# NomaDamas/AutoRAG-Research

Measured on AMD Instinct MI355X. Metric: queries/sec, higher is better.
Workload: dtype f32

## Files before the change

autorag_research_amd/csrc/dev_common.h:

```cpp
#pragma once
#include <hip/hip_runtime.h>
#include <stdint.h>

namespace mi355 {

constexpr int kWave = 64;
constexpr int kQBlockMax = 1024;
constexpr int kKMax = 1024;
constexpr int kCandCap = 2048;
constexpr int kCandCapWide = 4096;
constexpr int kSortMax = 4096;
constexpr int kIrrCap = 1024;
constexpr uint64_t kKeyNaN = 0xFFFFFFFFFFFFFFFFull;
static_assert(kSortMax >= kKMax + kCandCap, "the general prune's sort must hold k kept entries and a full candidate list");

constexpr int kStOverflow = 1;
constexpr int kStIrregular = 2;

struct QueryState {
    float* qn;
    uint16_t* qhat;
    float* thr;
    int* cnt;
    int* best_n;
// ... 191 lines not shown
__device__ __forceinline__ void bitonic_asc_key_row(uint64_t* key, int32_t* row, int n) {
    for (int k = 2; k <= n; k <<= 1) {
        for (int j = k >> 1; j > 0; j >>= 1) {
            for (int i = threadIdx.x; i < n; i += blockDim.x) {
                const int p = i ^ j;
                if (p > i) {
                    const bool asc = ((i & k) == 0);
                    const uint64_t ka = key[i], kb = key[p];
                    const int32_t ra = row[i], rb = row[p];
                    const bool a_after_b = key_before(kb, rb, ka, ra);
                    if (asc ? a_after_b : key_before(ka, ra, kb, rb)) {
                        key[i] = kb;
                        key[p] = ka;
                        row[i] = rb;
                        row[p] = ra;
                    }
                }
            }
            __syncthreads();
        }
    }
}

constexpr int kStageCols = 64;
constexpr int kStageLd = 68;
constexpr int kStageFloats = kWave * kStageLd;

__device__ __forceinline__ void wave_sync() {
    __builtin_amdgcn_fence(__ATOMIC_RELEASE, "wavefront");
    __builtin_amdgcn_wave_barrier();
    __builtin_amdgcn_fence(__ATOMIC_ACQUIRE, "wavefront");
}

typedef float f32x4_native __attribute__((ext_vector_type(4)));
typedef const f32x4_native __attribute__((address_space(1)))* gmem_f4;
__device__ __forceinline__ float4 load_gmem_f4(const float* p) {
    const f32x4_native v = *(gmem_f4)p;
    return make_float4(v.x, v.y, v.z, v.w);
}

struct StagePiece {
    float4 v[16];
};
struct StageRows {
    const float* r[16];
};
__device__ __forceinline__ void stage_rows_init(StageRows& sr, const float* my_row, int lane) {
    const unsigned long long a = (unsigned long long)my_row;
    const unsigned plo = (unsigned)(a & 0xFFFFFFFFull), phi = (unsigned)(a >> 32);
    const int sub = lane >> 4;
#pragma unroll
    for (int g = 0; g < 16; ++g) {
        const unsigned lo = __shfl(plo, g * 4 + sub, kWave), hi = __shfl(phi, g * 4 + sub, kWave);
        sr.r[g] = (const float*)(((unsigned long long)hi << 32) | lo);
    }
}

__device__ __forceinline__ bool stage_rows_init_dense(StageRows& sr, const float* my_row, int lane) {
    const unsigned long long live = __builtin_amdgcn_ballot_w64(my_row != nullptr);
    if (live == 0) {
        stage_rows_init(sr, my_row, lane);
        return false;
    }
    const int src = __builtin_ctzll(live);
    unsigned long long a = (unsigned long long)my_row;
    unsigned plo = (unsigned)(a & 0xFFFFFFFFull), phi = (unsigned)(a >> 32);
    const unsigned flo = __shfl(plo, src, kWave), fhi = __shfl(phi, src, kWave);
    if (my_row == nullptr) {
        plo = flo;
        phi = fhi;
    }
    const int sub = lane >> 4;
#pragma unroll
    for (int g = 0; g < 16; ++g) {
        const unsigned lo = __shfl(plo, g * 4 + sub, kWave), hi = __shfl(phi, g * 4 + sub, kWave);
        sr.r[g] = (const float*)(((unsigned long long)hi << 32) | lo);
    }
    return true;
}
__device__ __forceinline__ void stage_issue_dense(StagePiece& p, const StageRows& sr, int k0, int lane) {
    const int c4 = (lane & 15) * 4;
#pragma unroll
    for (int g = 0; g < 16; ++g) p.v[g] = load_gmem_f4(sr.r[g] + k0 + c4);
}

__device__ __forceinline__ void stage_issue(StagePiece& p, const StageRows& sr, int k0, int d, int lane) {
    const int c4 = (lane & 15) * 4;
#pragma unroll
    for (int g = 0; g < 16; ++g)
        p.v[g] = (sr.r[g] != nullptr && k0 + c4 < d) ? load_gmem_f4(sr.r[g] + k0 + c4) : make_float4(0.f, 0.f, 0.f, 0.f);
}
__device__ __forceinline__ void stage_commit(float* tile, const StagePiece& p, int lane) {
    wave_sync();
    const int sub = lane >> 4, c4 = (lane & 15) * 4;
#pragma unroll
    for (int g = 0; g < 16; ++g) *(float4*)(tile + (g * 4 + sub) * kStageLd + c4) = p.v[g];
    wave_sync();
}

__device__ __forceinline__ void stage_rows(float* tile, const float* my_row, int k0, int d, int lane) {
    if ((d & 3) == 0) {
        StageRows sr;
        StagePiece p;
        stage_rows_init(sr, my_row, lane);
        stage_issue(p, sr, k0, d, lane);
        stage_commit(tile, p, lane);
        return;
    }
    wave_sync();
    const unsigned long long a = (unsigned long long)my_row;
    const unsigned plo = (unsigned)(a & 0xFFFFFFFFull), phi = (unsigned)(a >> 32);
#pragma unroll 8
    for (int s = 0; s < kWave; ++s) {
        const unsigned lo = __shfl(plo, s, kWave), hi = __shfl(phi, s, kWave);
        const float* r = (const float*)(((unsigned long long)hi << 32) | lo);
        const int k = k0 + lane;
        tile[s * kStageLd + lane] = (r != nullptr && k < d) ? r[k] : 0.0f;
    }
    wave_sync();
}

__device__ __forceinline__ float chain_piece(const float* tile, int lane, const float* qv, int kn, float acc) {
    const float* t = tile + lane * kStageLd;
    if (kn == kStageCols) {
        float4 tv[16], q4[16];
#pragma unroll
        for (int i = 0; i < 16; ++i) {
            tv[i] = *(const float4*)(t + 4 * i);
            q4[i] = *(const float4*)(qv + 4 * i);
        }
#pragma unroll
        for (int i = 0; i < 16; ++i) {
            acc = __builtin_fmaf(tv[i].x, q4[i].x, acc);
            acc = __builtin_fmaf(tv[i].y, q4[i].y, acc);
            acc = __builtin_fmaf(tv[i].z, q4[i].z, acc);
            acc = __builtin_fmaf(tv[i].w, q4[i].w, acc);
        }
        return acc;
    }
    int k = 0;
    for (; k + 4 <= kn; k += 4) {
        const float4 tv = *(const float4*)(t + k);
        const float4 q4 = *(const float4*)(qv + k);
        acc = __builtin_fmaf(tv.x, q4.x, acc);
        acc = __builtin_fmaf(tv.y, q4.y, acc);
        acc = __builtin_fmaf(tv.z, q4.z, acc);
        acc = __builtin_fmaf(tv.w, q4.w, acc);
    }
    for (; k < kn; ++k) acc = __builtin_fmaf(t[k], qv[k], acc);
    return acc;
}

#ifndef MI355_STAGE_DEPTH
#define MI355_STAGE_DEPTH 2
#endif
template <int DEPTH = MI355_STAGE_DEPTH>
__device__ __forceinline__ float staged_dot(float* tile, const float* my_row, const float* qv, int d, int lane) {
    static_assert(DEPTH == 2 || DEPTH == 3, "pieces in flight");
    float acc = 0.0f;
    if ((d & 3) == 0) {
        StageRows sr;
        StagePiece p0, p1, p2;
        const bool dense = stage_rows_init_dense(sr, my_row, lane);
        auto issue = [&](StagePiece& p, int k0) __attribute__((always_inline)) {
            if (dense && k0 + kStageCols <= d) stage_issue_dense(p, sr, k0, lane);
            else stage_issue(p, sr, k0, d, lane);
        };
        issue(p0, 0);
        if (kStageCols < d) issue(p1, kStageCols);
        if constexpr (DEPTH == 3) {
            if (2 * kStageCols < d) issue(p2, 2 * kStageCols);
        }
        for (int k0 = 0; k0 < d; k0 += DEPTH * kStageCols) {
            stage_commit(tile, p0, lane);
            if (k0 + DEPTH * kStageCols < d) issue(p0, k0 + DEPTH * kStageCols);
            acc = chain_piece(tile, lane, qv + k0, min(kStageCols, d - k0), acc);
            if (k0 + kStageCols < d) {
                stage_commit(tile, p1, lane);
                if (k0 + (DEPTH + 1) * kStageCols < d) issue(p1, k0 + (DEPTH + 1) * kStageCols);
                acc = chain_piece(tile, lane, qv + k0 + kStageCols, min(kStageCols, d - k0 - kStageCols), acc);
            }
            if constexpr (DEPTH == 3) {
                if (k0 + 2 * kStageCols < d) {
                    stage_commit(tile, p2, lane);
                    if (k0 + 5 * kStageCols < d) issue(p2, k0 + 5 * kStageCols);
                    acc = chain_piece(tile, lane, qv + k0 + 2 * kStageCols, min(kStageCols, d - k0 - 2 * kStageCols), acc);
                }
            }
        }
    } else {
        for (int k0 = 0; k0 < d; k0 += kStageCols) {
            stage_rows(tile, my_row, k0, d, lane);
            acc = chain_piece(tile, lane, qv + k0, min(kStageCols, d - k0), acc);
        }
    }
    return acc;
}

__device__ __forceinline__ float chain_piece16(const float* tile, int lane, const float* qv, int kn_words, float acc) {
    const float* t = tile + lane * kStageLd;
    for (int w = 0; w + 4 <= kn_words; w += 4) {
        const uint4 tv = *(const uint4*)(t + w);
        const float4 qa = *(const float4*)(qv + 2 * w), qb = *(const float4*)(qv + 2 * w + 4);
        acc = __builtin_fmaf(__uint_as_float(tv.x << 16), qa.x, acc);
        acc = __builtin_fmaf(__uint_as_float(tv.x & 0xFFFF0000u), qa.y, acc);
        acc = __builtin_fmaf(__uint_as_float(tv.y << 16), qa.z, acc);
        acc = __builtin_fmaf(__uint_as_float(tv.y & 0xFFFF0000u), qa.w, acc);
        acc = __builtin_fmaf(__uint_as_float(tv.z << 16), qb.x, acc);
        acc = __builtin_fmaf(__uint_as_float(tv.z & 0xFFFF0000u), qb.y, acc);
        acc = __builtin_fmaf(__uint_as_float(tv.w << 16), qb.z, acc);
        acc = __builtin_fmaf(__uint_as_float(tv.w & 0xFFFF0000u), qb.w, acc);
    }
    return acc;
}
__device__ __forceinline__ float staged_dot16(float* tile, const float* my_row_words, const float* qv, int words, int lane) {
    float acc = 0.0f;
    StageRows sr;
    StagePiece p0, p1;
    stage_rows_init(sr, my_row_words, lane);
    stage_issue(p0, sr, 0, words, lane);
    if (kStageCols < words) stage_issue(p1, sr, kStageCols, words, lane);
    for (int k0 = 0; k0 < words; k0 += 2 * kStageCols) {
        stage_commit(tile, p0, lane);
        if (k0 + 2 * kStageCols < words) stage_issue(p0, sr, k0 + 2 * kStageCols, words, lane);
        acc = chain_piece16(tile, lane, qv + 2 * k0, min(kStageCols, words - k0), acc);
        if (k0 + kStageCols < words) {
            stage_commit(tile, p1, lane);
            if (k0 + 3 * kStageCols < words) stage_issue(p1, sr, k0 + 3 * kStageCols, words, lane);
            acc = chain_piece16(tile, lane, qv + 2 * (k0 + kStageCols), min(kStageCols, words - k0 - kStageCols), acc);
        }
    }
    return acc;
}

}
```

autorag_research_amd/csrc/k_select.h:

```cpp
#pragma once
#include "dev_common.h"

namespace mi355 {

struct PruneArgs {
    const float* rows;
    const float* nrm2;
    const float* q;
    QueryState st;
    int32_t* cand_row;
    float* cand_val;
    const int* qlist;
    unsigned long long* stat;
    int cap, d, k, metric;
    int exact;
    const uint8_t* flag8;
    float cscale;
    const uint16_t* shadow16;
    int dpad;
    int round_a;
    int* skip_list;
    int skip_parity;
    int thr_only;
    int one_wave_only;
// ... 159 lines not shown
        a.stat[2 * q] += (unsigned long long)(n_new - a.st.carry[q]);
        a.st.carry[q] = 0;
    }

    int n_res;
    int n_base = n_best;
    bool kept_loaded = false;
    if constexpr (THREADS == kWave) {
        if (!a.exact) {
            float* tile = tiles;
            uint32_t key[kSelPerLane];
            unsigned in_a = 0;
            load_candidate_keys<kSelPerLane, kWave>(key, cval, crow, a.flag8, n_new, lane);
            for (int k = lane; k < a.d; k += kWave) qs[k] = a.q[(int64_t)q * a.d + k];
            if (a.shadow16 != nullptr)
                for (int k = lane; k < a.dpad; k += kWave) q16[k] = bf16_bits_to_f32(a.st.qhat[(int64_t)q * a.dpad + k]);
            const int n_cand = wave_count_ge(key, 1u, n_new);
            auto rescore_list = [&](int n, int dst) __attribute__((always_inline)) {
                for (int base = 0; base < n; base += kWave) {
                    const int e = base + lane;
                    const bool live = e < n;
                    const int32_t row = live ? crow[R[e]] : -1;
                    const float* rp = live ? a.rows + (int64_t)row * a.d : nullptr;
                    const float acc = staged_dot(tile, rp, qs, a.d, lane);
                    if (live) {
                        int32_t kept = row;
                        SK[dst + e] = exact_key_of(a.metric, acc, nq, a.nrm2[row], kept);
                        SR[dst + e] = kept;
                    }
                }
            };
            auto compact = [&](uint32_t x, int room, bool mark) -> int {
                int n = 0;
#pragma unroll
                for (int j = 0; j < kSelPerLane; ++j) {
                    if (j * kWave >= n_new) break;
                    const bool want = key[j] >= x && key[j] != 0 && !((in_a >> j) & 1u);
                    const unsigned long long bal = __builtin_amdgcn_ballot_w64(want);
                    const int pos = n + (int)__builtin_amdgcn_mbcnt_hi((unsigned)(bal >> 32),
                                                                       __builtin_amdgcn_mbcnt_lo((unsigned)bal, 0));
                    if (want && pos < room) {
                        R[pos] = j * kWave + lane;
                        if (mark) in_a |= 1u << j;
                    }
                    n += __builtin_popcountll(bal);
                }
                return min(n, room);
// ... 52 lines not shown
                        }
                    }
                    asm volatile("s_waitcnt vmcnt(0)" ::: "memory");
#pragma unroll
                    for (int j = 0; j < kSelPerLane; ++j) {
                        if (j * kWave >= nB) break;
                        const int i = j * kWave + lane;
                        if (i < nB) {
                            crow_w[i] = cr[j];
                            cval_w[i] = cv[j];
                        }
                    }
                    carried = nB;
                    nB = 0;
                }
                if (a.shadow16 != nullptr && cut16 != -__builtin_inff() && nB > 0) {
                    const int words = a.dpad / 2;
                    int nS = 0;
                    for (int base = 0; base < nB; base += kWave) {
                        const int e = base + lane;
                        const bool live = e < nB;
                        const int ci = live ? R[e] : 0;
                        const float* rp = live ? (const float*)(a.shadow16 + (int64_t)crow[ci] * a.dpad) : nullptr;
                        const float t16 = staged_dot16(tile, rp, q16, words, lane);
                        const bool keep = live && !(t16 < cut16);
                        const unsigned long long bal = __builtin_amdgcn_ballot_w64(keep);
                        const int pos = nS + (int)__builtin_amdgcn_mbcnt_hi((unsigned)(bal >> 32),
                                                                           __builtin_amdgcn_mbcnt_lo((unsigned)bal, 0));
                        wave_sync();
                        if (keep) R[pos] = ci;
                        nS += __builtin_popcountll(bal);
                    }
                    nB = nS;
                    wave_sync();
                }
                rescore_list(nB, n1);
            }
            if (lane == 0) a.stat[2 * q + 1] += (unsigned long long)(nA + nB);
            wave_sync();
            const int n_tot = n1 + nB;
            uint64_t* K2 = (uint64_t*)X;
            int32_t* R2 = (int32_t*)(X + (size_t)SORT * 8);
            int n_sel = n_tot;
            if (n_tot > a.k) {
                uint32_t sk[kSelPerLane];
#pragma unroll
                for (int j = 0; j < kSelPerLane; ++j) {
// ... 275 lines not shown
```

autorag_research_amd/csrc/mi355dr.hip:

```cpp
#include "index.h"
#include "k_prep.h"
#include "k_scan.h"
#include "k_scan_ids.h"
#include "subset_ids.h"
#include "screen_common.h"
#include "k_screen.h"
#include "k_screen256c.h"
#include "k_screen_rq.h"

#define MI355_RQ_FORMS(X) X(1) X(2) X(3) X(4) X(5) X(6)
inline bool screen_rq_has(int ksteps) { return ksteps >= 1 && ksteps <= 6; }
#include "k_screen_stream.h"
#include "k_select.h"
#include "k_prune_wide.h"
#include "k_update.h"
#include "k_compact.h"
#include "k_view.h"
#include "k_block.h"
#include "k_mmr.h"
#include "mmr_order.h"
#include "k_groups.h"
#include "k_range.h"
#include "k_rows.h"

// ... 195 lines not shown
}

inline bool i8_available(const mi355dr_index* idx) { return idx->irr8_n <= kIrrCap; }
Pass decide_pass(const mi355dr_index* idx, int k, int level, bool force_scan, const char* no_screen = nullptr) {
    Pass ps;
    ps.k = k;
    ps.level = level;
    const int path = force_scan ? (int)MI355DR_PATH_SCAN : idx->path;
    if (level > 0) ps.i8 = false;
    else if (idx->screen_dtype == MI355DR_SCREEN_I8) ps.i8 = true;
    else ps.i8 = idx->screen_dtype == MI355DR_SCREEN_AUTO && i8_available(idx) && k < idx->i8_demoted_k &&
                 growth_budget(idx, k, true) >= idx->i8_min_budget;
    const bool screen_possible = ps.i8 ? i8_available(idx) : idx->irr_n <= kIrrCap;
    ps.screening = idx->n > 0 && screen_possible && path != MI355DR_PATH_SCAN;
    ps.wide = ps.screening && wide_ok(idx, k);
    ps.cap = !idx->cap_set && ps.wide ? kCandCapWide : idx->cap;
    if (idx->screen_dtype == MI355DR_SCREEN_I8 && !i8_available(idx) && path != MI355DR_PATH_SCAN)
        ps.refused = "int8 screen unavailable: too many rows outside the residual limit";
    else if (path == MI355DR_PATH_SCREEN && !screen_possible && idx->n > 0) ps.refused = no_screen;
    return ps;
}
inline bool idle_i8(const mi355dr_index* idx) { return decide_pass(idx, idx->last_pass_k, 0, false).i8; }

int launch_prune(mi355dr_index* idx, hipStream_t s, const Pass& ps, int nblocks, const int* qlist, int exact,
                 bool thr_only = false, bool one_wave_only = false, bool defer_b = false) {
    PruneArgs pa{};
    pa.thr_only = thr_only ? 1 : 0;
    pa.one_wave_only = one_wave_only ? 1 : 0;
    pa.defer_b = defer_b && idx->defer_round_b ? 1 : 0;
    pa.rows = idx->rows;
    pa.nrm2 = idx->nrm2;
    pa.q = idx->qdev;
    pa.st = idx->st;
    pa.cand_row = idx->cand_row;
    pa.cand_val = idx->cand_val;
    pa.qlist = qlist;
    pa.stat = idx->stat_dev;
    pa.cap = ps.cap;
    pa.d = idx->dim;
    pa.k = ps.k;
    pa.metric = idx->metric;
    pa.exact = exact;
    pa.flag8 = (ps.i8 && (idx->irr8_n > 0 || idx->dead_n > 0)) ? idx->flag8 : nullptr;
    pa.cscale = idx->metric == MI355DR_METRIC_IP ? idx->cmax : 1.0f;
    pa.shadow16 = (ps.i8 && idx->metric == 0 && !exact && idx->prefilter16) ? idx->shadow : nullptr;
    pa.dpad = idx->dpad;
    pa.round_a = idx->round_a;
    if (!exact && ps.wide) {
        pa.shadow16 = nullptr;
        hipLaunchKernelGGL((k_prune_wide<2, 32>), dim3(nblocks), dim3(2 * kWave), prune_wide_lds_bytes(idx->dim, 2), s, pa);
        HIPCHECK(idx, hipGetLastError());
        return MI355DR_OK;
    }
    if (pa.cap > kCandCap) return fail(idx, MI355DR_E_INTERNAL, "general-form prune on a list stride above kCandCap");
    const bool list_mode = qlist == nullptr;
    pa.skip_list = list_mode ? idx->prune_skip : nullptr;
    pa.skip_parity = list_mode ? (idx->prune_parity ^= 1) : 0;
    hipLaunchKernelGGL((k_prune<kPruneSmallThreads, kPruneSmallSort>), dim3(nblocks), dim3(kPruneSmallThreads),
                       prune_lds_bytes(idx->dim, kPruneSmallThreads, kPruneSmallSort, pa.shadow16 ? idx->dpad : 0), s, pa);
    HIPCHECK(idx, hipGetLastError());
    if (one_wave_only) return MI355DR_OK;
    hipLaunchKernelGGL((k_prune<kPruneBigThreads, kPruneBigSort>), dim3(list_mode ? std::min(nblocks, 64) : nblocks),
                       dim3(kPruneBigThreads), prune_lds_bytes(idx->dim, kPruneBigThreads, kPruneBigSort, 0), s, pa);
    HIPCHECK(idx, hipGetLastError());
    return MI355DR_OK;
}

int launch_prep(mi355dr_index* idx, hipStream_t s, int B, int Bpad, int metric, bool i8, int cnt0 = 0) {
    hipLaunchKernelGGL(k_prep_queries, dim3(Bpad), dim3(64), (size_t)idx->dim * sizeof(float), s, idx->qdev, B, idx->dim,
                       idx->dpad, metric, idx->st, idx->dpad8, i8 ? 1 : 0, idx->bf16_ec, idx->status_or_dev,
                       idx->prune_skip, cnt0, idx->metric == MI355DR_METRIC_IP ? idx->cmax : 1.0f);
    idx->prune_parity = 0;
    HIPCHECK(idx, hipGetLastError());
    return MI355DR_OK;
}

inline int screen_tile(int B) { return B > kTileN ? kT2 : kTileM; }

constexpr int kRetryLevels = 2;

enum ScreenKernel { kKernTile = 0, kKernStream = 1, kKern256c = 2, kKernRq = 3 };
inline ScreenKernel screen_kernel_for(const mi355dr_index* idx, bool i8, int B, int64_t rows, bool emit_all) {
    const int tile = (emit_all || rows <= idx->small_chunk_rows) ? kTileM : screen_tile(B);
    const int row_bytes = i8 ? idx->dpad8 : idx->dpad * 2;
    const int ksteps = row_bytes / kRowB;
    if (tile == kT2) return i8 && idx->screen_rq && screen_rq_has(ksteps) ? kKernRq : kKern256c;
    if (!emit_all && idx->screen_stream && B <= 64 && ksteps >= 1 && (B <= 32 ? 32 : 64) * row_bytes <= kStreamQueryBytesMax)
        return kKernStream;
    return kKernTile;
}

int launch_screen(mi355dr_index* idx, hipStream_t s, bool i8, int B, int64_t r0, int64_t r_end, int cap, int emit_mode,
// ... 134 lines not shown
            const int64_t len = end - prev;
            if (len >= 2 * round_rows) end = std::min<int64_t>(n, prev + (len + round_rows / 2) / round_rows * round_rows);
        }
        if (end <= prev) continue;
        p.ends.push_back(end);
        prev = end;
        if (end >= n) break;
    }
    if (p.ends.empty() || p.ends.back() < n) p.ends.push_back(n);
    return p;
}

inline int starter_count(const PassPlan& p) { return (int)((p.sample + kSlabRows - 1) / kSlabRows); }

PassPlan make_plan(const mi355dr_index* idx, const Pass& ps, int B) {
    const double budget = growth_budget(idx, ps.k, ps.i8);
    double growth = std::max(0.25, std::min((double)idx->chunk_growth, budget));
    if (B <= 64 && ps.level == 0 && idx->chunk_growth_set == 0) growth = std::max(growth, std::min(8.0, budget * kSmallBlockBudget));
    if (ps.level == 1) growth = std::max(0.25, growth * 0.5);
    if (ps.level >= 2) growth = 0.25;
    return plan_pass(idx, ps, B, growth);
}

int run_screen(mi355dr_index* idx, hipStream_t s, const Pass& ps, int B, const PassPlan& plan) {
    int64_t kept_all_below = 0;
    const bool i8 = ps.i8;
    const int side_n = i8 ? idx->irr8_n : idx->irr_n;
    constexpr int kSideMerge = 32;
    bool side_done = false;
    const bool lean = plan.sample > 0 && idx->prune_companion == 0;
    auto timed = [&](bool big, int64_t rows, auto&& launch) -> int {
        EventPair ev{};
        if (idx->profile) {
            ev = take_events(idx);
            HIPCHECK(idx, hipEventRecord(ev.a, s));
        }
        CHECK(launch());
        if (idx->profile) {
            HIPCHECK(idx, hipEventRecord(ev.b, s));
            ev.big = big ? 1 : 0;
            idx->ev_pending.v.push_back(ev);
        }
        idx->s_screen_launches++;
        idx->s_screen_rows += rows;
        if (big) {
            idx->s_big_launches++;
            idx->s_big_rows += rows;
        }
        return MI355DR_OK;
    };
    if (plan.sample > 0) {
        CHECK(timed(false, plan.sample, [&] { return launch_screen(idx, s, i8, B, 0, plan.sample, ps.cap, kEmitSlabMax, -1); }));
        CHECK(launch_prune(idx, s, ps, B, nullptr, 0, true, true));
        idx->s_starters++;
    }
    int64_t done = 0;
    for (size_t ci = 0; ci < plan.ends.size(); ++ci) {
        const int64_t end = plan.ends[ci];
        const bool emit_all = ci == 0 && plan.emit_all_first;
        if (emit_all) kept_all_below = end;
        const bool big = !emit_all && end - done > idx->small_chunk_rows && screen_tile(B) == kT2;
        const int64_t seen = ci == 0 ? (plan.sample > 0 ? plan.sample : end) : done;
        const double lanes = 8.0 * ps.k * 4096.0 / (double)std::max<int64_t>(seen, 1);
        int period = 1;
        while (period < 64 && period * 2 * lanes <= idx->screen_flush_lanes) period *= 2;
        const int flush_mask = idx->screen_flush_sync ? period - 1 : -1;
        CHECK(timed(big, end - done, [&] { return launch_screen(idx, s, i8, B, done, end, ps.cap, emit_all ? kEmitAll : 0, flush_mask); }));
        idx->s_chunks++;
        if (end >= idx->n && side_n > 0 && side_n <= kSideMerge) {
            hipLaunchKernelGGL(k_emit_irregular, dim3(B), dim3(64), 0, s, i8 ? idx->irr8_rows : idx->irr_rows, side_n, idx->st,
                               idx->cand_row, idx->cand_val, ps.cap, (int)kept_all_below);
            HIPCHECK(idx, hipGetLastError());
            side_done = true;
        }
        const bool last = end >= idx->n && (side_n == 0 || side_done);
        CHECK(launch_prune(idx, s, ps, B, nullptr, 0, false, lean, !last));
        done = end;
    }
    if (side_n > 0 && !side_done) {
        hipLaunchKernelGGL(k_emit_irregular, dim3(B), dim3(64), 0, s, i8 ? idx->irr8_rows : idx->irr_rows, side_n, idx->st,
                           idx->cand_row, idx->cand_val, ps.cap, (int)kept_all_below);
        HIPCHECK(idx, hipGetLastError());
        CHECK(launch_prune(idx, s, ps, B, nullptr, 0, false, lean));
    }
    idx->s_passes++;
    return MI355DR_OK;
}

int launch_scan(mi355dr_index* idx, hipStream_t s, const int* qlist, int nq, int cap, int64_t r0, int64_t r1,
                const int32_t* ids = nullptr) {
    ScanArgs sa{};
    sa.rows = idx->rows;
    sa.nrm2 = idx->nrm2;
    sa.q = idx->qdev;
    sa.st = idx->st;
    sa.cand_row = idx->cand_row;
    sa.cand_val = idx->cand_val;
    sa.qlist = qlist;
    sa.nq = nq;
    sa.cap = cap;
    sa.d = idx->dim;
    sa.metric = idx->metric;
    sa.row0 = r0;
    sa.row1 = r1;
    const dim3 grid((unsigned)((r1 - r0 + kScanThreads - 1) / kScanThreads));
    const ScanIdsArgs ia{sa, ids};
    if (ids) hipLaunchKernelGGL(k_scan_ids, grid, dim3(kScanThreads), scan_ids_lds_bytes(idx->dim, nq), s, ia);
    else if (idx->dim % kScan32PieceCols == 0 && idx->scan_dma)
        hipLaunchKernelGGL(k_scan32, grid, dim3(kScanThreads), kScan32Lds, s, sa, idx->n);
    else hipLaunchKernelGGL(k_scan, grid, dim3(kScanThreads), scan_lds_bytes(idx->dim, nq), s, sa);
    HIPCHECK(idx, hipGetLastError());
    return MI355DR_OK;
}

int scan_range(mi355dr_index* idx, hipStream_t s, const Pass& ps, int off, int nq, int64_t r0, int64_t r1, const int32_t* ids) {
    CHECK(launch_scan(idx, s, idx->qlist_dev + off, nq, ps.cap, r0, r1, ids));
    return launch_prune(idx, s, ps, nq, idx->qlist_dev + off, 1);
}

int run_scan(mi355dr_index* idx, hipStream_t s, const Pass& ps, const std::vector<int>& qs, int64_t total,
             const int32_t* ids = nullptr) {
    if (qs.empty()) return MI355DR_OK;
    HIPCHECK(idx, hipMemcpyAsync(idx->qlist_dev, qs.data(), qs.size() * sizeof(int), hipMemcpyHostToDevice, s));
    const int nq_all = (int)qs.size(), cap = ps.cap;
    hipLaunchKernelGGL(k_reset_queries, dim3((nq_all + 255) / 256), dim3(256), 0, s, idx->st, idx->qlist_dev, nq_all);
    HIPCHECK(idx, hipGetLastError());
    const int per = kScanQ;
    for (int off = 0; off < nq_all; off += per) {
        const int nq = std::min(per, nq_all - off);
        int64_t done = 0;
        int64_t chunk = std::min<int64_t>(idx->chunk0_rows, cap);
        while (done < total) {
            const int64_t end = std::min<int64_t>(total, done + chunk);
            CHECK(scan_range(idx, s, ps, off, nq, done, end, ids));
            if (end - done > cap) {
                HIPCHECK(idx, hipMemcpyAsync(idx->status_host, idx->st.status, kQBlockMax * sizeof(int),
                                             hipMemcpyDeviceToHost, s));
                HIPCHECK(idx, hipStreamSynchronize(s));
                std::vector<int> redo;
                for (int j = 0; j < nq; ++j)
// ... 9 lines not shown
                    for (int64_t p = done; p < end; p += cap)
                        CHECK(scan_range(idx, s, ps, roff, (int)redo.size(), p, std::min<int64_t>(end, p + cap), ids));
                    if (ids) {
                        HIPCHECK(idx, hipStreamSynchronize(s));
                        idx->s_subset_rerun_queries += (int64_t)redo.size();
                    }
                }
            }
            done = end;
            chunk = std::max<int64_t>(chunk, done * (idx->chunk_growth_set ? idx->chunk_growth : 63));
        }
    }
    if (ids) HIPCHECK(idx, hipStreamSynchronize(s));
    else idx->s_fallback_queries += nq_all;
    return MI355DR_OK;
}

int subset_block(mi355dr_index* idx, hipStream_t s, const float* q_dev, int B, int k, int64_t m, double* out_dist_dev,
                 int64_t* out_rows_dev) {
    const Pass ps = decide_pass(idx, k, 0, true);
    idx->last_pass_k = k;
    if (q_dev != idx->qdev)
        HIPCHECK(idx, hipMemcpyAsync(idx->qdev, q_dev, (size_t)B * idx->dim * sizeof(float), hipMemcpyDeviceToDevice, s));
    CHECK(launch_prep(idx, s, B, (int)round_up(B, screen_tile(B)), idx->metric, ps.i8));
    std::vector<int> all(B);
    for (int i = 0; i < B; ++i) all[i] = i;
    if (m > 0) CHECK(run_scan(idx, s, ps, all, m, idx->subset_ids));
    hipLaunchKernelGGL(k_finalize, dim3(B), dim3(64), 0, s, idx->st, k, idx->row_offset, idx->view_row_map.p, out_dist_dev,
                       out_rows_dev, idx->status_or_dev);
    HIPCHECK(idx, hipGetLastError());
    HIPCHECK(idx, hipMemcpyAsync(idx->status_host, idx->st.status, (size_t)kQBlockMax * sizeof(int), hipMemcpyDeviceToHost, s));
    HIPCHECK(idx, hipStreamSynchronize(s));
    for (int i = 0; i < B; ++i)
        if (idx->status_host[i] & kStOverflow)
            return fail(idx, MI355DR_E_INTERNAL, "subset scan: query " + std::to_string(i) + " lost a candidate chunk");
    return MI355DR_OK;
}

int pending_alloc(mi355dr_index* idx, Pending& p) {
    HIPCHECK(idx, p.status_host.grow((kQBlockMax + 1) * sizeof(int)));
    HIPCHECK(idx, p.done.create(hipEventDisableTiming));
    return MI355DR_OK;
}

int enqueue_block(mi355dr_index* idx, hipStream_t s, const float* q_dev, int B, int k, double* out_dist_dev,
                  int64_t* out_rows_dev, Pending& p, int level = 0, bool force_scan = false) {
    CHECK(ensure_qstate(idx));
    CHECK(pending_alloc(idx, p));
    idx->last_pass_k = k;
    if (level == 0 && idx->screen_dtype == MI355DR_SCREEN_AUTO && k >= idx->i8_demoted_k && --idx->i8_probation <= 0)
        idx->i8_demoted_k = INT_MAX;
    const int Bpad = (int)round_up(B, screen_tile(B));
    const Pass ps = decide_pass(idx, k, level, force_scan, "screen path unavailable (metric or too many irregular rows)");
    if (ps.refused) return fail(idx, MI355DR_E_UNSUPPORTED, ps.refused);
    if (q_dev != idx->qdev)
        HIPCHECK(idx, hipMemcpyAsync(idx->qdev, q_dev, (size_t)B * idx->dim * sizeof(float), hipMemcpyDeviceToDevice, s));
    PassPlan plan;
    if (ps.screening) plan = make_plan(idx, ps, B);
    CHECK(launch_prep(idx, s, B, Bpad, idx->metric, ps.i8, starter_count(plan)));
    if (idx->n > 0) {
        if (ps.screening) {
            CHECK(run_screen(idx, s, ps, B, plan));
        } else {
            std::vector<int> all(B);
            for (int i = 0; i < B; ++i) all[i] = i;
            CHECK(run_scan(idx, s, ps, all, idx->n));
        }
    }
    hipLaunchKernelGGL(k_finalize, dim3(B), dim3(64), 0, s, idx->st, k, idx->row_offset, idx->view_row_map.p, out_dist_dev,
                       out_rows_dev, idx->status_or_dev);
    HIPCHECK(idx, hipGetLastError());
    HIPCHECK(idx, hipMemcpyAsync(p.status_host, idx->st.status, (size_t)(kQBlockMax + 1) * sizeof(int), hipMemcpyDeviceToHost, s));
    HIPCHECK(idx, hipEventRecord(p.done, s));
    p.active = true;
    p.stream = s;
    p.q_dev = q_dev;
    p.B = B;
    p.pass = ps;
    p.out_dist = out_dist_dev;
    p.out_rows = out_rows_dev;
    return MI355DR_OK;
}

int search_block(mi355dr_index* idx, hipStream_t s, const float* q_dev, int B, int k, double* out_dist_dev,
                 int64_t* out_rows_dev, int level = 0, bool force_scan = false);
// ... 77 lines not shown
    return np * 12;
}
inline int merge_threads(int world, int k) { return (int64_t)world * k <= 128 ? 64 : 256; }

int launch_merge(mi355dr_index* idx, const double* dist_all, const int64_t* rows_all, int64_t stride, int world, int B, int k,
                 double* out_dist_dev, int64_t* out_rows_dev, void* stream) {
    if (world <= 0 || B < 0 || k <= 0) return fail(idx, MI355DR_E_INVALID, "bad merge shape");
    if ((int64_t)world * k > kSortMax) return fail(idx, MI355DR_E_UNSUPPORTED, "world*k exceeds 4096");
    if (B == 0) return MI355DR_OK;
    HIPCHECK(idx, hipSetDevice(idx->device));
    CHECK(ensure_qstate(idx));
    hipStream_t s = stream ? (hipStream_t)stream : idx->stream;
    hipLaunchKernelGGL(k_merge_topk, dim3(B), dim3(merge_threads(world, k)), merge_lds(world, k), s, dist_all, rows_all, stride,
                       world, B, k, out_dist_dev, out_rows_dev);
    HIPCHECK(idx, hipGetLastError());
    return MI355DR_OK;
}

int upload_and_prep(mi355dr_index* idx, const float* queries, int B, int metric) {
    HIPCHECK(idx, hipSetDevice(idx->device));
    CHECK(drain_pending(idx));
    CHECK(ensure_qstate(idx));
    HIPCHECK(idx, hipMemcpyAsync(idx->qdev, queries, (size_t)B * idx->dim * sizeof(float), hipMemcpyHostToDevice, idx->stream));
    return launch_prep(idx, idx->stream, B, (int)round_up(B, screen_tile(B)), metric, idle_i8(idx));
}

int check_search_args(mi355dr_index* idx, const void* q, int B, int k, const void* od, const void* orow) {
    if (!idx) return fail(nullptr, MI355DR_E_INVALID, "null index");
    if (B < 0 || k <= 0) return fail(idx, MI355DR_E_INVALID, "B must be >= 0 and k > 0");
    if (k > kKMax) return fail(idx, MI355DR_E_UNSUPPORTED, "k exceeds 1024");
    if (B > 0 && (!q || !od || !orow)) return fail(idx, MI355DR_E_INVALID, "null buffer");
    return MI355DR_OK;
}

int check_radii(mi355dr_index* idx, const std::string& what, const double* radius, int B) {
    for (int b = 0; b < B; ++b)
        if (radius[b] != radius[b]) return fail(idx, MI355DR_E_INVALID, what + ": radius " + std::to_string(b) + " is NaN");
    return MI355DR_OK;
}

enum : unsigned { kCallNoView = 1, kCallDrain = 2 };
struct Call {
    std::unique_lock<std::mutex> lock;
    hipStream_t s = nullptr;
};
template <class ArgCheck>
int begin_call(mi355dr_index* idx, const char* what, void* stream, unsigned flags, Call& c, ArgCheck&& args_ok) {
// ... 995 lines not shown
        const int nq = std::min(kScanQ, nq_all - off);
        CHECK(launch_scan(idx, s, idx->qlist_dev + off, nq, ps.cap, r0, r1));
        CHECK(launch_range_collect(idx, s, ps, rs, kRangeFormExact, nq, idx->qlist_dev + off, span, r0));
    }
    return MI355DR_OK;
}

int range_block(mi355dr_index* idx, hipStream_t s, const float* q_dev, int nb, const double* radius, int m, double* od,
                int64_t* orow, int64_t* ocount) {
    const Pass ps = decide_pass(idx, 1, 0, false, "screen path unavailable (too many irregular rows)");
    if (ps.refused) return fail(idx, MI355DR_E_UNSUPPORTED, ps.refused);
    const int cap = ps.cap;
    const bool i8 = ps.i8, use_screen = ps.screening;
    const int64_t chunk = round_up(std::max<int64_t>(idx->range_chunk_rows, kT2), kT2);
    std::vector<RangeSpan> spans;
    for (int64_t r0 = 0; r0 < idx->n; r0 += chunk) spans.push_back(RangeSpan{r0, std::min(idx->n, r0 + chunk)});
    const int n_main = (int)spans.size();
    const int R = range_slots_for(idx, m);
    const int64_t pairs = (int64_t)nb * std::max(n_main, 1);
    CHECK(ensure_range(idx, nb, R, m, pairs));
    const RangeState rs = range_state(idx, R, pairs);
    if (q_dev != idx->qdev)
        HIPCHECK(idx, hipMemcpyAsync(idx->qdev, q_dev, (size_t)nb * idx->dim * sizeof(float), hipMemcpyDeviceToDevice, s));
    CHECK(launch_prep(idx, s, nb, (int)round_up(nb, screen_tile(nb)), idx->metric, i8));
    HIPCHECK(idx, hipMemcpyAsync(idx->rng.radius.p, radius, (size_t)nb * sizeof(double), hipMemcpyHostToDevice, s));
    HIPCHECK(idx, hipMemsetAsync(idx->rng.redo.p, 0, 2 * sizeof(int), s));
    HIPCHECK(idx, hipMemsetAsync(idx->rng.stat.p, 0, 2 * sizeof(unsigned long long), s));
    hipLaunchKernelGGL(k_range_prep, dim3((nb + kRangeThreads - 1) / kRangeThreads), dim3(kRangeThreads), 0, s,
                       (const double*)idx->rng.radius.p, nb, idx->metric, use_screen ? 1 : 0, idx->st, rs);
    HIPCHECK(idx, hipGetLastError());
    std::vector<int> all(nb);
    for (int i = 0; i < nb; ++i) all[i] = i;
    if (use_screen) {
        for (int i = 0; i < n_main; ++i) {
            CHECK(launch_screen(idx, s, i8, nb, spans[i].r0, spans[i].r1, cap, 0, idx->screen_flush_sync ? 15 : -1));
            CHECK(launch_range_collect(idx, s, ps, rs, kRangeFormScreen, nb, nullptr, i, spans[i].r0));
        }
        const int side_n = i8 ? idx->irr8_n : idx->irr_n;
        const int32_t* side = i8 ? idx->irr8_rows.p : idx->irr_rows.p;
        for (int i0 = 0; i0 < side_n; i0 += cap) {
            hipLaunchKernelGGL(k_emit_irregular, dim3(nb), dim3(64), 0, s, side + i0, std::min(cap, side_n - i0), idx->st,
                               idx->cand_row, idx->cand_val, cap, 0);
            HIPCHECK(idx, hipGetLastError());
            CHECK(launch_range_collect(idx, s, ps, rs, kRangeFormSide, nb, nullptr, -1, 0));
        }
    } else if (n_main > 0) {
        HIPCHECK(idx, hipMemcpyAsync(idx->qlist_dev, all.data(), (size_t)nb * sizeof(int), hipMemcpyHostToDevice, s));
// ... 126 lines not shown
    }));
    if (B == 0) return MI355DR_OK;
    hipStream_t s = c.s;
    HIPCHECK(idx, idx->rowq.reserve(std::min(B, kQBlockMax), stride, idx->dim, range));
    HIPCHECK(idx, hipMemsetAsync(idx->rowq.skipped_dev.p, 0, sizeof(unsigned long long), s));
    const CallIO<> io{host, s, nullptr, {out_dist, out_rows, out_count}, kout};
    std::vector<double> rad;
    for (int b0 = 0; b0 < B; b0 += kQBlockMax) {
        const int nb = std::min(kQBlockMax, B - b0);
        const BlockOut<int64_t> o = block_outputs(idx, io, b0);
        HIPCHECK(idx, hipMemcpyAsync(idx->rowq.ids.p, row_ids + b0, (size_t)nb * sizeof(int64_t), hipMemcpyHostToDevice, s));
        hipLaunchKernelGGL(k_rows_gather, dim3(nb), dim3(kRowsThreads), 0, s, (const int64_t*)idx->rowq.ids.p, idx->row_offset,
                           idx->n, (const float*)idx->rows.p, (const float*)idx->nrm2.p, idx->dim, idx->rowq.q.p,
                           idx->rowq.valid.p, idx->rowq.pair_q.p, idx->rowq.pair_row.p, idx->rowq.skipped_dev.p);
        HIPCHECK(idx, hipGetLastError());
        if (idx->n > 0 && !range) {
            CHECK(search_block(idx, s, idx->rowq.q.p, nb, stride, idx->rowq.cand_dist.p, idx->rowq.cand_rows.p));
        } else if (idx->n > 0) {
            rad.assign(radius + b0, radius + b0 + nb);
            for (int b = 0; b < nb; ++b)
                if (subset_local_row(row_ids[b0 + b], idx->row_offset, idx->n) < 0) rad[b] = -INFINITY;
            HIPCHECK(idx, hipMemcpyAsync(idx->rowq.radius.p, rad.data(), (size_t)nb * sizeof(double), hipMemcpyHostToDevice, s));
            HIPCHECK(idx, hipMemcpyAsync(idx->qdev, idx->rowq.q.p, (size_t)nb * idx->dim * sizeof(float), hipMemcpyDeviceToDevice, s));
            CHECK(launch_prep(idx, s, nb, (int)round_up(nb, screen_tile(nb)), idx->metric, idle_i8(idx)));
            CHECK(launch_rescore(idx, s, idx->rowq.pair_q.p, idx->rowq.pair_row.p, nb, idx->rowq.self_dot.p, idx->rowq.self_dist.p));
            CHECK(range_block(idx, s, idx->rowq.q.p, nb, rad.data(), stride, idx->rowq.cand_dist.p, idx->rowq.cand_rows.p,
                              idx->rowq.cand_count.p));
        }
        hipLaunchKernelGGL(k_rows_drop, dim3(nb), dim3(kRowsThreads), 0, s, (const double*)idx->rowq.cand_dist.p,
                           (const int64_t*)idx->rowq.cand_rows.p, stride, (const int64_t*)idx->rowq.ids.p,
                           (const int*)idx->rowq.valid.p, kout, include_self ? 1 : 0,
                           range ? (const int64_t*)idx->rowq.cand_count.p : nullptr, (const double*)idx->rowq.self_dist.p,
                           (const double*)idx->rowq.radius.p, o.dist, o.rows, o.count);
        HIPCHECK(idx, hipGetLastError());
        CHECK(block_return(idx, io, b0, nb, o));
        HIPCHECK(idx, hipStreamSynchronize(s));
    }
    unsigned long long skipped = 0;
    HIPCHECK(idx, hipMemcpy(&skipped, idx->rowq.skipped_dev.p, sizeof(skipped), hipMemcpyDeviceToHost));
    idx->s_rows_searches++;
    idx->s_rows_queries += B;
    idx->s_rows_skipped += (int64_t)skipped;
    return MI355DR_OK;
}
}

int mi355dr_search_rows(mi355dr_index* idx, const int64_t* row_ids, int B, int k, int flags, double* out_dist, int64_t* out_rows) {
// ... 431 lines not shown
```

Baseline: 160,200.

## Stage wider, fewer-row tiles when a prune wave has few live candidates

Adds StageGeom geometries (16 or 32 rows with wider columns) so that partially filled waves in the exact and bf16 prune stages load fewer rows per piece but cover more columns. This is meant to cut the number of staging iterations and the wasted loads on dead lanes when few candidates remain. The cost is idle lanes during the dot chain and extra code paths. It also removes the depth-3 staging option, and in the screening path it reads queries straight from q_dev instead of first copying them into qdev.

```diff
diff --git a/autorag_research_amd/csrc/dev_common.h b/autorag_research_amd/csrc/dev_common.h
--- a/autorag_research_amd/csrc/dev_common.h
+++ b/autorag_research_amd/csrc/dev_common.h
@@ -237,9 +237,40 @@
     }
 }
 
-constexpr int kStageCols = 64;
-constexpr int kStageLd = 68;
+template <int R>
+struct StageGeom {
+    static_assert(R == 64 || R == 32 || R == 16, "row slots of a piece");
+    static constexpr int kRows = R;
+    static constexpr int kCols = kWave * 64 / R;
+    static constexpr int kLd = kCols + 4;
+    static constexpr int kLanesPerRow = kCols / 4;
+    static constexpr int kRowsPerLoad = kWave / kLanesPerRow;
+    static constexpr int row(int g, int lane) { return g * kRowsPerLoad + lane / kLanesPerRow; }
+    static constexpr int col(int lane) { return 4 * (lane % kLanesPerRow); }
+    static constexpr bool covers_once() {
+        bool seen[kRows * kLanesPerRow] = {};
+        for (int g = 0; g < 16; ++g)
+            for (int lane = 0; lane < kWave; ++lane) {
+                const int r = row(g, lane), c = col(lane);
+                if (r < 0 || r >= kRows || c < 0 || c + 4 > kCols || seen[r * kLanesPerRow + c / 4]) return false;
+                seen[r * kLanesPerRow + c / 4] = true;
+            }
+        for (int i = 0; i < kRows * kLanesPerRow; ++i)
+            if (!seen[i]) return false;
+        return true;
+    }
+};
+constexpr int kStageCols = StageGeom<64>::kCols;
+constexpr int kStageLd = StageGeom<64>::kLd;
 constexpr int kStageFloats = kWave * kStageLd;
+static_assert(kStageCols == 64 && kStageLd == 68, "the full-batch geometry");
+static_assert(StageGeom<64>::kRows * StageGeom<64>::kLd <= kStageFloats && StageGeom<32>::kRows * StageGeom<32>::kLd <= kStageFloats &&
+                  StageGeom<16>::kRows * StageGeom<16>::kLd <= kStageFloats,
+              "a geometry's tile exceeds the tile buffer");
+static_assert(StageGeom<64>::kLd % 64 == 4 && StageGeom<32>::kLd % 64 == 4 && StageGeom<16>::kLd % 64 == 4,
+              "row stride: 1 mod 16 sixteen-byte slots");
+static_assert(StageGeom<64>::covers_once() && StageGeom<32>::covers_once() && StageGeom<16>::covers_once(),
+              "lane <-> (row, column) map of a piece");
 
 __device__ __forceinline__ void wave_sync() {
     __builtin_amdgcn_fence(__ATOMIC_RELEASE, "wavefront");
@@ -260,21 +291,23 @@
 struct StageRows {
     const float* r[16];
 };
+template <int R = 64>
 __device__ __forceinline__ void stage_rows_init(StageRows& sr, const float* my_row, int lane) {
     const unsigned long long a = (unsigned long long)my_row;
     const unsigned plo = (unsigned)(a & 0xFFFFFFFFull), phi = (unsigned)(a >> 32);
-    const int sub = lane >> 4;
 #pragma unroll
     for (int g = 0; g < 16; ++g) {
-        const unsigned lo = __shfl(plo, g * 4 + sub, kWave), hi = __shfl(phi, g * 4 + sub, kWave);
+        const int src = StageGeom<R>::row(g, lane);
+        const unsigned lo = __shfl(plo, src, kWave), hi = __shfl(phi, src, kWave);
         sr.r[g] = (const float*)(((unsigned long long)hi << 32) | lo);
     }
 }
 
+template <int R = 64>
 __device__ __forceinline__ bool stage_rows_init_dense(StageRows& sr, const float* my_row, int lane) {
     const unsigned long long live = __builtin_amdgcn_ballot_w64(my_row != nullptr);
     if (live == 0) {
-        stage_rows_init(sr, my_row, lane);
+        stage_rows_init<R>(sr, my_row, lane);
         return false;
     }
     const int src = __builtin_ctzll(live);
@@ -285,31 +318,33 @@
         plo = flo;
         phi = fhi;
     }
-    const int sub = lane >> 4;
 #pragma unroll
     for (int g = 0; g < 16; ++g) {
-        const unsigned lo = __shfl(plo, g * 4 + sub, kWave), hi = __shfl(phi, g * 4 + sub, kWave);
+        const int from = StageGeom<R>::row(g, lane);
+        const unsigned lo = __shfl(plo, from, kWave), hi = __shfl(phi, from, kWave);
         sr.r[g] = (const float*)(((unsigned long long)hi << 32) | lo);
     }
     return true;
 }
+template <int R = 64>
 __device__ __forceinline__ void stage_issue_dense(StagePiece& p, const StageRows& sr, int k0, int lane) {
-    const int c4 = (lane & 15) * 4;
+    const int c4 = StageGeom<R>::col(lane);
 #pragma unroll
     for (int g = 0; g < 16; ++g) p.v[g] = load_gmem_f4(sr.r[g] + k0 + c4);
 }
 
 __device__ __forceinline__ void stage_issue(StagePiece& p, const StageRows& sr, int k0, int d, int lane) {
-    const int c4 = (lane & 15) * 4;
+    const int c4 = StageGeom<64>::col(lane);
 #pragma unroll
     for (int g = 0; g < 16; ++g)
         p.v[g] = (sr.r[g] != nullptr && k0 + c4 < d) ? load_gmem_f4(sr.r[g] + k0 + c4) : make_float4(0.f, 0.f, 0.f, 0.f);
 }
+template <int R = 64>
 __device__ __forceinline__ void stage_commit(float* tile, const StagePiece& p, int lane) {
     wave_sync();
-    const int sub = lane >> 4, c4 = (lane & 15) * 4;
-#pragma unroll
-    for (int g = 0; g < 16; ++g) *(float4*)(tile + (g * 4 + sub) * kStageLd + c4) = p.v[g];
+    const int c4 = StageGeom<R>::col(lane);
+#pragma unroll
+    for (int g = 0; g < 16; ++g) *(float4*)(tile + StageGeom<R>::row(g, lane) * StageGeom<R>::kLd + c4) = p.v[g];
     wave_sync();
 }
 
@@ -335,8 +370,7 @@
     wave_sync();
 }
 
-__device__ __forceinline__ float chain_piece(const float* tile, int lane, const float* qv, int kn, float acc) {
-    const float* t = tile + lane * kStageLd;
+__device__ __forceinline__ float chain_row(const float* t, const float* qv, int kn, float acc) {
     if (kn == kStageCols) {
         float4 tv[16], q4[16];
 #pragma unroll
@@ -365,17 +399,31 @@
     for (; k < kn; ++k) acc = __builtin_fmaf(t[k], qv[k], acc);
     return acc;
 }
-
-#ifndef MI355_STAGE_DEPTH
-#define MI355_STAGE_DEPTH 2
-#endif
-template <int DEPTH = MI355_STAGE_DEPTH>
+__device__ __forceinline__ float chain_piece(const float* tile, int lane, const float* qv, int kn, float acc) {
+    return chain_row(tile + lane * kStageLd, qv, kn, acc);
+}
+template <int R>
+__device__ __forceinline__ float chain_piece_wide(const float* tile, int lane, const float* qv, float acc) {
+    using G = StageGeom<R>;
+    if (lane < R) {
+        const float* t = tile + lane * G::kLd;
+#pragma unroll 1
+        for (int c = 0; c < G::kCols; c += kStageCols) acc = chain_row(t + c, qv + c, kStageCols, acc);
+    }
+    return acc;
+}
+
+__device__ __forceinline__ int stage_geom_rows(int n_live, int len) {
+    if (n_live <= 16 && len % StageGeom<16>::kCols == 0) return 16;
+    if (n_live <= 32 && len % StageGeom<32>::kCols == 0) return 32;
+    return 64;
+}
+
 __device__ __forceinline__ float staged_dot(float* tile, const float* my_row, const float* qv, int d, int lane) {
-    static_assert(DEPTH == 2 || DEPTH == 3, "pieces in flight");
     float acc = 0.0f;
     if ((d & 3) == 0) {
         StageRows sr;
-        StagePiece p0, p1, p2;
+        StagePiece p0, p1;
         const bool dense = stage_rows_init_dense(sr, my_row, lane);
         auto issue = [&](StagePiece& p, int k0) __attribute__((always_inline)) {
             if (dense && k0 + kStageCols <= d) stage_issue_dense(p, sr, k0, lane);
@@ -383,24 +431,14 @@
         };
         issue(p0, 0);
         if (kStageCols < d) issue(p1, kStageCols);
-        if constexpr (DEPTH == 3) {
-            if (2 * kStageCols < d) issue(p2, 2 * kStageCols);
-        }
-        for (int k0 = 0; k0 < d; k0 += DEPTH * kStageCols) {
+        for (int k0 = 0; k0 < d; k0 += 2 * kStageCols) {
             stage_commit(tile, p0, lane);
-            if (k0 + DEPTH * kStageCols < d) issue(p0, k0 + DEPTH * kStageCols);
+            if (k0 + 2 * kStageCols < d) issue(p0, k0 + 2 * kStageCols);
             acc = chain_piece(tile, lane, qv + k0, min(kStageCols, d - k0), acc);
             if (k0 + kStageCols < d) {
                 stage_commit(tile, p1, lane);
-                if (k0 + (DEPTH + 1) * kStageCols < d) issue(p1, k0 + (DEPTH + 1) * kStageCols);
+                if (k0 + 3 * kStageCols < d) issue(p1, k0 + 3 * kStageCols);
                 acc = chain_piece(tile, lane, qv + k0 + kStageCols, min(kStageCols, d - k0 - kStageCols), acc);
-            }
-            if constexpr (DEPTH == 3) {
-                if (k0 + 2 * kStageCols < d) {
-                    stage_commit(tile, p2, lane);
-                    if (k0 + 5 * kStageCols < d) issue(p2, k0 + 5 * kStageCols);
-                    acc = chain_piece(tile, lane, qv + k0 + 2 * kStageCols, min(kStageCols, d - k0 - 2 * kStageCols), acc);
-                }
             }
         }
     } else {
@@ -411,9 +449,35 @@
     }
     return acc;
 }
-
-__device__ __forceinline__ float chain_piece16(const float* tile, int lane, const float* qv, int kn_words, float acc) {
-    const float* t = tile + lane * kStageLd;
+template <int R>
+__device__ __forceinline__ float staged_dot_wide(float* tile, const float* my_row, const float* qv, int d, int lane) {
+    using G = StageGeom<R>;
+    float acc = 0.0f;
+    StageRows sr;
+    StagePiece p0, p1;
+    stage_rows_init_dense<R>(sr, my_row, lane);
+    stage_issue_dense<R>(p0, sr, 0, lane);
+    if (G::kCols < d) stage_issue_dense<R>(p1, sr, G::kCols, lane);
+    for (int k0 = 0; k0 < d; k0 += 2 * G::kCols) {
+        stage_commit<R>(tile, p0, lane);
+        if (k0 + 2 * G::kCols < d) stage_issue_dense<R>(p0, sr, k0 + 2 * G::kCols, lane);
+        acc = chain_piece_wide<R>(tile, lane, qv + k0, acc);
+        if (k0 + G::kCols < d) {
+            stage_commit<R>(tile, p1, lane);
+            if (k0 + 3 * G::kCols < d) stage_issue_dense<R>(p1, sr, k0 + 3 * G::kCols, lane);
+            acc = chain_piece_wide<R>(tile, lane, qv + k0 + G::kCols, acc);
+        }
+    }
+    return acc;
+}
+__device__ __forceinline__ float staged_dot(float* tile, const float* my_row, const float* qv, int d, int lane, int n_live) {
+    const int rows = stage_geom_rows(n_live, d);
+    if (rows == 16) return staged_dot_wide<16>(tile, my_row, qv, d, lane);
+    if (rows == 32) return staged_dot_wide<32>(tile, my_row, qv, d, lane);
+    return staged_dot(tile, my_row, qv, d, lane);
+}
+
+__device__ __forceinline__ float chain_row16(const float* t, const float* qv, int kn_words, float acc) {
     for (int w = 0; w + 4 <= kn_words; w += 4) {
         const uint4 tv = *(const uint4*)(t + w);
         const float4 qa = *(const float4*)(qv + 2 * w), qb = *(const float4*)(qv + 2 * w + 4);
@@ -427,6 +491,9 @@
         acc = __builtin_fmaf(__uint_as_float(tv.w & 0xFFFF0000u), qb.w, acc);
     }
     return acc;
+}
+__device__ __forceinline__ float chain_piece16(const float* tile, int lane, const float* qv, int kn_words, float acc) {
+    return chain_row16(tile + lane * kStageLd, qv, kn_words, acc);
 }
 __device__ __forceinline__ float staged_dot16(float* tile, const float* my_row_words, const float* qv, int words, int lane) {
     float acc = 0.0f;
@@ -447,5 +514,36 @@
     }
     return acc;
 }
-
-}
+template <int R>
+__device__ __forceinline__ float staged_dot16_wide(float* tile, const float* my_row_words, const float* qv, int words, int lane) {
+    using G = StageGeom<R>;
+    float acc = 0.0f;
+    StageRows sr;
+    StagePiece p0, p1;
+    stage_rows_init_dense<R>(sr, my_row_words, lane);
+    stage_issue_dense<R>(p0, sr, 0, lane);
+    if (G::kCols < words) stage_issue_dense<R>(p1, sr, G::kCols, lane);
+    auto chain = [&](int k0) __attribute__((always_inline)) {
+        if (lane < R) acc = chain_row16(tile + lane * G::kLd, qv + 2 * k0, G::kCols, acc);
+    };
+    for (int k0 = 0; k0 < words; k0 += 2 * G::kCols) {
+        stage_commit<R>(tile, p0, lane);
+        if (k0 + 2 * G::kCols < words) stage_issue_dense<R>(p0, sr, k0 + 2 * G::kCols, lane);
+        chain(k0);
+        if (k0 + G::kCols < words) {
+            stage_commit<R>(tile, p1, lane);
+            if (k0 + 3 * G::kCols < words) stage_issue_dense<R>(p1, sr, k0 + 3 * G::kCols, lane);
+            chain(k0 + G::kCols);
+        }
+    }
+    return acc;
+}
+__device__ __forceinline__ float staged_dot16(float* tile, const float* my_row_words, const float* qv, int words, int lane,
+                                              int n_live) {
+    const int rows = stage_geom_rows(n_live, words);
+    if (rows == 16) return staged_dot16_wide<16>(tile, my_row_words, qv, words, lane);
+    if (rows == 32) return staged_dot16_wide<32>(tile, my_row_words, qv, words, lane);
+    return staged_dot16(tile, my_row_words, qv, words, lane);
+}
+
+}
diff --git a/autorag_research_amd/csrc/k_select.h b/autorag_research_amd/csrc/k_select.h
--- a/autorag_research_amd/csrc/k_select.h
+++ b/autorag_research_amd/csrc/k_select.h
@@ -205,7 +205,7 @@
                     const bool live = e < n;
                     const int32_t row = live ? crow[R[e]] : -1;
                     const float* rp = live ? a.rows + (int64_t)row * a.d : nullptr;
-                    const float acc = staged_dot(tile, rp, qs, a.d, lane);
+                    const float acc = staged_dot(tile, rp, qs, a.d, lane, min(kWave, n - base));
                     if (live) {
                         int32_t kept = row;
                         SK[dst + e] = exact_key_of(a.metric, acc, nq, a.nrm2[row], kept);
@@ -304,7 +304,7 @@
                         const bool live = e < nB;
                         const int ci = live ? R[e] : 0;
                         const float* rp = live ? (const float*)(a.shadow16 + (int64_t)crow[ci] * a.dpad) : nullptr;
-                        const float t16 = staged_dot16(tile, rp, q16, words, lane);
+                        const float t16 = staged_dot16(tile, rp, q16, words, lane, min(kWave, nB - base));
                         const bool keep = live && !(t16 < cut16);
                         const unsigned long long bal = __builtin_amdgcn_ballot_w64(keep);
                         const int pos = nS + (int)__builtin_amdgcn_mbcnt_hi((unsigned)(bal >> 32),
diff --git a/autorag_research_amd/csrc/mi355dr.hip b/autorag_research_amd/csrc/mi355dr.hip
--- a/autorag_research_amd/csrc/mi355dr.hip
+++ b/autorag_research_amd/csrc/mi355dr.hip
@@ -241,7 +241,7 @@
 }
 inline bool idle_i8(const mi355dr_index* idx) { return decide_pass(idx, idx->last_pass_k, 0, false).i8; }
 
-int launch_prune(mi355dr_index* idx, hipStream_t s, const Pass& ps, int nblocks, const int* qlist, int exact,
+int launch_prune(mi355dr_index* idx, hipStream_t s, const Pass& ps, const float* q, int nblocks, const int* qlist, int exact,
                  bool thr_only = false, bool one_wave_only = false, bool defer_b = false) {
     PruneArgs pa{};
     pa.thr_only = thr_only ? 1 : 0;
@@ -249,7 +249,7 @@
     pa.defer_b = defer_b && idx->defer_round_b ? 1 : 0;
     pa.rows = idx->rows;
     pa.nrm2 = idx->nrm2;
-    pa.q = idx->qdev;
+    pa.q = q;
     pa.st = idx->st;
     pa.cand_row = idx->cand_row;
     pa.cand_val = idx->cand_val;
@@ -285,8 +285,8 @@
     return MI355DR_OK;
 }
 
-int launch_prep(mi355dr_index* idx, hipStream_t s, int B, int Bpad, int metric, bool i8, int cnt0 = 0) {
-    hipLaunchKernelGGL(k_prep_queries, dim3(Bpad), dim3(64), (size_t)idx->dim * sizeof(float), s, idx->qdev, B, idx->dim,
+int launch_prep(mi355dr_index* idx, hipStream_t s, const float* q, int B, int Bpad, int metric, bool i8, int cnt0 = 0) {
+    hipLaunchKernelGGL(k_prep_queries, dim3(Bpad), dim3(64), (size_t)idx->dim * sizeof(float), s, q, B, idx->dim,
                        idx->dpad, metric, idx->st, idx->dpad8, i8 ? 1 : 0, idx->bf16_ec, idx->status_or_dev,
                        idx->prune_skip, cnt0, idx->metric == MI355DR_METRIC_IP ? idx->cmax : 1.0f);
     idx->prune_parity = 0;
@@ -467,7 +467,7 @@
     return plan_pass(idx, ps, B, growth);
 }
 
-int run_screen(mi355dr_index* idx, hipStream_t s, const Pass& ps, int B, const PassPlan& plan) {
+int run_screen(mi355dr_index* idx, hipStream_t s, const Pass& ps, const float* q, int B, const PassPlan& plan) {
     int64_t kept_all_below = 0;
     const bool i8 = ps.i8;
     const int side_n = i8 ? idx->irr8_n : idx->irr_n;
@@ -496,7 +496,7 @@
     };
     if (plan.sample > 0) {
         CHECK(timed(false, plan.sample, [&] { return launch_screen(idx, s, i8, B, 0, plan.sample, ps.cap, kEmitSlabMax, -1); }));
-        CHECK(launch_prune(idx, s, ps, B, nullptr, 0, true, true));
+        CHECK(launch_prune(idx, s, ps, q, B, nullptr, 0, true, true));
         idx->s_starters++;
     }
     int64_t done = 0;
@@ -519,14 +519,14 @@
             side_done = true;
         }
         const bool last = end >= idx->n && (side_n == 0 || side_done);
-        CHECK(launch_prune(idx, s, ps, B, nullptr, 0, false, lean, !last));
+        CHECK(launch_prune(idx, s, ps, q, B, nullptr, 0, false, lean, !last));
         done = end;
     }
     if (side_n > 0 && !side_done) {
         hipLaunchKernelGGL(k_emit_irregular, dim3(B), dim3(64), 0, s, i8 ? idx->irr8_rows : idx->irr_rows, side_n, idx->st,
                            idx->cand_row, idx->cand_val, ps.cap, (int)kept_all_below);
         HIPCHECK(idx, hipGetLastError());
-        CHECK(launch_prune(idx, s, ps, B, nullptr, 0, false, lean));
+        CHECK(launch_prune(idx, s, ps, q, B, nullptr, 0, false, lean));
     }
     idx->s_passes++;
     return MI355DR_OK;
@@ -560,7 +560,7 @@
 
 int scan_range(mi355dr_index* idx, hipStream_t s, const Pass& ps, int off, int nq, int64_t r0, int64_t r1, const int32_t* ids) {
     CHECK(launch_scan(idx, s, idx->qlist_dev + off, nq, ps.cap, r0, r1, ids));
-    return launch_prune(idx, s, ps, nq, idx->qlist_dev + off, 1);
+    return launch_prune(idx, s, ps, idx->qdev, nq, idx->qlist_dev + off, 1);
 }
 
 int run_scan(mi355dr_index* idx, hipStream_t s, const Pass& ps, const std::vector<int>& qs, int64_t total,
@@ -616,7 +616,7 @@
     idx->last_pass_k = k;
     if (q_dev != idx->qdev)
         HIPCHECK(idx, hipMemcpyAsync(idx->qdev, q_dev, (size_t)B * idx->dim * sizeof(float), hipMemcpyDeviceToDevice, s));
-    CHECK(launch_prep(idx, s, B, (int)round_up(B, screen_tile(B)), idx->metric, ps.i8));
+    CHECK(launch_prep(idx, s, idx->qdev, B, (int)round_up(B, screen_tile(B)), idx->metric, ps.i8));
     std::vector<int> all(B);
     for (int i = 0; i < B; ++i) all[i] = i;
     if (m > 0) CHECK(run_scan(idx, s, ps, all, m, idx->subset_ids));
@@ -647,14 +647,15 @@
     const int Bpad = (int)round_up(B, screen_tile(B));
     const Pass ps = decide_pass(idx, k, level, force_scan, "screen path unavailable (metric or too many irregular rows)");
     if (ps.refused) return fail(idx, MI355DR_E_UNSUPPORTED, ps.refused);
-    if (q_dev != idx->qdev)
+    const float* q = ps.screening ? q_dev : idx->qdev.p;
+    if (q != q_dev)
         HIPCHECK(idx, hipMemcpyAsync(idx->qdev, q_dev, (size_t)B * idx->dim * sizeof(float), hipMemcpyDeviceToDevice, s));
     PassPlan plan;
     if (ps.screening) plan = make_plan(idx, ps, B);
-    CHECK(launch_prep(idx, s, B, Bpad, idx->metric, ps.i8, starter_count(plan)));
+    CHECK(launch_prep(idx, s, q, B, Bpad, idx->metric, ps.i8, starter_count(plan)));
     if (idx->n > 0) {
         if (ps.screening) {
-            CHECK(run_screen(idx, s, ps, B, plan));
+            CHECK(run_screen(idx, s, ps, q, B, plan));
         } else {
             std::vector<int> all(B);
             for (int i = 0; i < B; ++i) all[i] = i;
@@ -778,7 +779,7 @@
     CHECK(drain_pending(idx));
     CHECK(ensure_qstate(idx));
     HIPCHECK(idx, hipMemcpyAsync(idx->qdev, queries, (size_t)B * idx->dim * sizeof(float), hipMemcpyHostToDevice, idx->stream));
-    return launch_prep(idx, idx->stream, B, (int)round_up(B, screen_tile(B)), metric, idle_i8(idx));
+    return launch_prep(idx, idx->stream, idx->qdev, B, (int)round_up(B, screen_tile(B)), metric, idle_i8(idx));
 }
 
 int check_search_args(mi355dr_index* idx, const void* q, int B, int k, const void* od, const void* orow) {
@@ -1820,7 +1821,7 @@
     const RangeState rs = range_state(idx, R, pairs);
     if (q_dev != idx->qdev)
         HIPCHECK(idx, hipMemcpyAsync(idx->qdev, q_dev, (size_t)nb * idx->dim * sizeof(float), hipMemcpyDeviceToDevice, s));
-    CHECK(launch_prep(idx, s, nb, (int)round_up(nb, screen_tile(nb)), idx->metric, i8));
+    CHECK(launch_prep(idx, s, idx->qdev, nb, (int)round_up(nb, screen_tile(nb)), idx->metric, i8));
     HIPCHECK(idx, hipMemcpyAsync(idx->rng.radius.p, radius, (size_t)nb * sizeof(double), hipMemcpyHostToDevice, s));
     HIPCHECK(idx, hipMemsetAsync(idx->rng.redo.p, 0, 2 * sizeof(int), s));
     HIPCHECK(idx, hipMemsetAsync(idx->rng.stat.p, 0, 2 * sizeof(unsigned long long), s));
@@ -1993,7 +1994,7 @@
                 if (subset_local_row(row_ids[b0 + b], idx->row_offset, idx->n) < 0) rad[b] = -INFINITY;
             HIPCHECK(idx, hipMemcpyAsync(idx->rowq.radius.p, rad.data(), (size_t)nb * sizeof(double), hipMemcpyHostToDevice, s));
             HIPCHECK(idx, hipMemcpyAsync(idx->qdev, idx->rowq.q.p, (size_t)nb * idx->dim * sizeof(float), hipMemcpyDeviceToDevice, s));
-            CHECK(launch_prep(idx, s, nb, (int)round_up(nb, screen_tile(nb)), idx->metric, idle_i8(idx)));
+            CHECK(launch_prep(idx, s, idx->qdev, nb, (int)round_up(nb, screen_tile(nb)), idx->metric, idle_i8(idx)));
             CHECK(launch_rescore(idx, s, idx->rowq.pair_q.p, idx->rowq.pair_row.p, nb, idx->rowq.self_dot.p, idx->rowq.self_dist.p));
             CHECK(range_block(idx, s, idx->rowq.q.p, nb, rad.data(), stride, idx->rowq.cand_dist.p, idx->rowq.cand_rows.p,
                               idx->rowq.cand_count.p));
```

Measured after the change: 160,600, median of 6. Within noise of the previous version (+0.2%).
